# GuildOfWeavers/distaff

Hardware: AMD Instinct MI355X
Metric: trace_cells_per_sec (higher is better)
Workload: dtype u128 (prime field 2^128-45*2^40+1, 4x u32 limbs)

## Files before the change

### distaff_amd/csrc/kernels_ntt.hip

```cpp
#include "ctx.h"
#include <mutex>
#include <type_traits>
#include "ntt_lds.h"

#if defined(NTT_NO_ROTATE)
#define NTT_NO_ROTATE_DEFINED 1
#else
#define NTT_NO_ROTATE_DEFINED 0
#endif
#define NTT_TILE_ELEMS 4096

struct NttArgs {
    const fe* src; fe* dst;
    size_t src_col_stride, src_coset_stride;
    size_t dst_col_stride, dst_coset_stride;
    const fe_tw* stage_tw;
    const fe_tw* prescale;
    const fe_tw* dit_last;
    const tw4_t* tw4;
    size_t tw4_coset_stride;
    uint32_t log_n1, log_n2, tile , log_N, log_b;
    uint32_t j0;
    uint32_t has_scale;
    uint32_t tiles_per_block;
    uint32_t debug;
    size_t src_row_stride, dst_k_stride, src_batch_stride, dst_batch_stride;
    uint32_t batch_log;
    uint32_t dit;
    uint32_t groups, cosets, cols;
    uint32_t coset_fast;
    uint32_t pre;
    const fe_tw* pre_tw;
    fe_tw scale;
};

__device__ __forceinline__ fe load_fe(const fe* p) { return *p; }

__device__ __forceinline__ fe dom_pow(const fe* lo, const fe* hi, uint32_t lo_bits, uint64_t e) {
    uint32_t l = (uint32_t)e & ((1u << lo_bits) - 1u), h = (uint32_t)(e >> lo_bits);
    fe a = lo[l];
    if (h == 0) return a;
    return fe_mul(a, hi[h]);
}

__device__ __forceinline__ void ntt_block(const NttArgs& a, uint32_t& group, uint32_t& jl, uint32_t& col) {
    const uint32_t b = blockIdx.x, units = a.groups * a.cosets;
    uint32_t u;
    if (a.coset_fast) {
        const uint32_t s = b >> 3, pairs = a.cosets * a.cols, pair = s % pairs;
        group = (s / pairs) * 8u + (b & 7u);
        const uint32_t chunk = pair / (4u * a.cosets), in_chunk = pair - chunk * 4u * a.cosets;
        const uint32_t width = (chunk * 4u + 4u <= a.cols) ? 4u : a.cols - chunk * 4u;
        col = chunk * 4u + in_chunk % width; jl = in_chunk / width;
        return;
    }
    if ((units & 7u) == 0) { const uint32_t s = b >> 3; col = s % a.cols; u = (s / a.cols) * 8u + (b & 7u); }
    else { col = b % a.cols; u = b / a.cols; }
    jl = u / a.groups; group = u % a.groups;
}

struct OutB {
    static constexpr bool active = true;
    fe* __restrict__ dst ; uint32_t k_stride, log_n2; bool scale; fe_tw s;
    uint32_t pre_shift, h;
    struct Tok {};
    __device__ __forceinline__ Tok pre(uint32_t, uint32_t) const { return Tok{}; }
    __device__ __forceinline__ void put(uint32_t row, uint32_t t, const fe& v, const Tok&) const {
        const uint32_t k2 = ((log_n2 ? (__brev(row) >> (32 - log_n2)) : 0u) << pre_shift) + h;
#if NTT_STREAM_B_STORE
        fe_store_stream(dst + (k2 * k_stride + t), scale ? fe_mul_tw(v, s) : v);
#else
        dst[k2 * k_stride + t] = scale ? fe_mul_tw(v, s) : v;
#endif
    }
};

#ifndef NTT_STREAM_STORE
#define NTT_STREAM_STORE 1
#endif
#ifndef NTT_STREAM_B_STORE
#define NTT_STREAM_B_STORE 1
#endif
#ifndef NTT_STREAM_B_LOAD
#define NTT_STREAM_B_LOAD 1
#endif
#if defined(NTT_LAB_SRC_SMALL)
#define NTT_LAB_SRC(row, t, off) ((((NTT_LAB_SRC_SMALL) == 1) || hh) ? ((((row) & 1023u) << 2) + ((t) & 3u)) : (off))
#else
#define NTT_LAB_SRC(row, t, off) (off)
#endif
#if defined(NTT_LAB_TW4_SMALL)
#define NTT_LAB_TW(row, t, off) ((((row) & 1023u) << 2) + ((t) & 3u))
#else
#define NTT_LAB_TW(row, t, off) (off)
#endif
#if defined(NTT_LAB_STAMPS)
#define NTT_LAB_WG_STRIDE 61u
__device__ unsigned long long ntt_lab_buf[2 * 256 * 16 * 2 * 16];
extern "C" __attribute__((visibility("default"))) int dst_lab_stamps(unsigned long long* out, size_t count, int clear) {
    if (count > sizeof(ntt_lab_buf) / 8) return -1;
    if (hipMemcpyFromSymbol(out, HIP_SYMBOL(ntt_lab_buf), count * 8) != hipSuccess) return -2;
    if (clear) { static unsigned long long zero[2 * 256 * 16 * 2 * 16]; if (hipMemcpyToSymbol(HIP_SYMBOL(ntt_lab_buf), zero, sizeof zero) != hipSuccess) return -3; }
    return 0;
}
#define NTT_LAB_FLUSH(pass, it, st, nst) do { \
    if ((blockIdx.x % NTT_LAB_WG_STRIDE) == 0u && blockIdx.x / NTT_LAB_WG_STRIDE < 256u && (it) < 2u && (threadIdx.x & 63u) == 0u) { \
        unsigned long long* o_ = ntt_lab_buf + ((((size_t)(pass) * 256u + blockIdx.x / NTT_LAB_WG_STRIDE) * 16u + (threadIdx.x >> 6)) * 2u + (it)) * 16u; \
        for (int k_ = 0; k_ < (nst); k_++) o_[k_] = (st)[k_]; } } while (0)
#else
#define NTT_LAB_FLUSH(pass, it, st, nst) ((void)0)
#endif
extern __shared__ __attribute__((aligned(16))) unsigned char ntt_smem[];

template <int THREADS, int WPE = 4, bool PREFETCH = true, int LOG_LEN = 0, int LOG_T = 0, int PRE = 0>
__global__ void __launch_bounds__(THREADS, WPE) ntt_pass_a(NttArgs a, const fe* __restrict__ src_base, fe* __restrict__ dst_base) {
    constexpr int EPT = NTT_TILE_ELEMS / THREADS;
    fe* L = reinterpret_cast<fe*>(ntt_smem);
    const uint32_t log_n1 = LOG_LEN ? (uint32_t)LOG_LEN : a.log_n1;
    const uint32_t log_t = LOG_T ? (uint32_t)LOG_T : a.tile, T = 1u << log_t, n1 = 1u << log_n1;
    fe_tw* TW = reinterpret_cast<fe_tw*>(L + n1 * T);
    uint32_t group, jl, col;
    ntt_block(a, group, jl, col);
    uint32_t hh = 0;
    if (PRE) { const uint32_t half = a.groups >> 1; hh = group >= half ? 1u : 0u; group -= hh * half; }
    const uint32_t jg = a.j0 + jl;
    const fe* __restrict__ src0 = src_base + (size_t)col * a.src_col_stride + (size_t)jl * a.src_coset_stride;
    fe* __restrict__ dst0 = dst_base + (size_t)col * a.dst_col_stride + (size_t)jl * a.dst_coset_stride;
    const uint32_t pmask = (1u << (a.log_b + log_n1 + PRE)) - 1u;
    const uint32_t jv = jg + (hh << a.log_b);
    if (a.dit) {
        const uint32_t in_lds = a.dit_last ? n1 / 2 : n1;
        for (uint32_t i = threadIdx.x; i + 1 < in_lds; i += THREADS) {
            const uint32_t lb = 31u - (uint32_t)__clz(i + 1), k = i + 1 - (1u << lb);
            TW[i] = a.prescale[((jv + (k << (a.log_b + PRE))) << (log_n1 - lb - 1)) & pmask];
        }
    } else
    for (uint32_t i = threadIdx.x; i < n1 / 2; i += THREADS) TW[dif_tw_slot(i)] = a.stage_tw[i];
    const bool scaled = !a.dit && a.prescale != nullptr && jg != 0;
    fe pre0 = fe_zero(), pre1 = fe_zero(), pre2 = fe_zero(), pre3 = fe_zero(), pre4 = fe_zero(), pre5 = fe_zero(), pre6 = fe_zero(), pre7 = fe_zero();
    const uint32_t count = n1 * T;
#define NTT_EACH(M) { M(0, pre0) M(1, pre1) M(2, pre2) M(3, pre3) M(4, pre4) M(5, pre5) M(6, pre6) M(7, pre7) }
    const bool rot_a = a.dit && log_t == 2 && !NTT_NO_ROTATE_DEFINED;
#define NTT_COL_A(idx) (rot_a ? (((idx) + ((idx) >> log_t)) & (T - 1)) : ((idx) & (T - 1)))
    const fe_tw pre_c = (PRE && a.dit) ? a.prescale[(jg << log_n1) & pmask] : fe_tw{};
    auto pre_stage_a = [&](const fe& x0, const fe& x1, uint32_t row) -> fe {
        if (a.dit) { const fe t = fe_mul_tw(x1, pre_c); return hh ? fe_sub(x0, t) : fe_add(x0, t); }
        return hh ? fe_mul_tw(fe_sub(x0, x1), a.pre_tw[row]) : fe_add(x0, x1);
    };
#define NTT_FETCH_A1(e, var) if constexpr ((e) < EPT) { uint32_t idx = lane + (e) * THREADS; idx = idx < count ? idx : 0u; \
        if constexpr (PRE != 0) { const uint32_t row_ = idx >> log_t; const fe x0_ = src[NTT_LAB_SRC(row_, NTT_COL_A(idx), (row_ << a.log_n2) + NTT_COL_A(idx))], x1_ = src[NTT_LAB_SRC(row_ + 512u, NTT_COL_A(idx), ((row_ + n1) << a.log_n2) + NTT_COL_A(idx))]; var = pre_stage_a(x0_, x1_, row_); } \
        else var = src[NTT_LAB_SRC(idx >> log_t, NTT_COL_A(idx), ((idx >> log_t) << a.log_n2) + NTT_COL_A(idx))]; }
#define NTT_FETCH_A(tile) { const fe* __restrict__ src = src0 + (tile) * T; NTT_EACH(NTT_FETCH_A1) }
    const tw4_t* __restrict__ tw4 = a.tw4 + (size_t)jl * a.tw4_coset_stride;
    const uint32_t tile0 = group * a.tiles_per_block;
    uint32_t lane = threadIdx.x;
    if (PREFETCH) NTT_FETCH_A(tile0)
    for (uint32_t it = 0; it < a.tiles_per_block; it++) {
        const uint32_t tile = tile0 + it;
        unsigned long long st[16]; (void)st;
        NTT_STAMP_REAL(st, 14);
        NTT_STAMP(st, 8);
        lane = lds_opaque_lane();
        if (!PREFETCH) NTT_FETCH_A(tile)
        NTT_STAMP(st, 9);
        __syncthreads();
        NTT_STAMP(st, 10);
#define NTT_PUT_A(e, var) if constexpr ((e) < EPT) { const uint32_t idx = lane + (e) * THREADS; if (idx < count) { if (a.dit) L[lds_slot(__brev(idx >> log_t) >> (32 - log_n1), NTT_COL_A(idx), log_t)] = var; else L[lds_slot(idx >> log_t, idx & (T - 1), log_t)] = scaled ? fe_mul_tw(var, a.prescale[(jg * (idx >> log_t)) & pmask]) : var; } }
        NTT_EACH(NTT_PUT_A)
#undef NTT_PUT_A
        NTT_STAMP(st, 11);
        __syncthreads();
        NTT_STAMP(st, 12);
        if (PREFETCH && it + 1 < a.tiles_per_block) NTT_FETCH_A(tile + 1)
        if constexpr (LOG_LEN != 0) {
            if (a.dit) lds_ntt_dit_fixed<THREADS, LOG_LEN, LOG_T>(L, TW, a.dit_last ? a.dit_last + (size_t)((jg << PRE) + hh) * (n1 / 2) : nullptr, NttKeepInLds(), st);
            else lds_ntt_dif_fixed<THREADS, LOG_LEN, LOG_T>(L, TW, NttKeepInLds(), st);
        } else {
            if (a.dit) lds_ntt_dit<THREADS>(L, TW, log_n1, log_t, 1u, log_n1 + 1u, a.dit_last ? a.dit_last + (size_t)((jg << PRE) + hh) * (n1 / 2) : nullptr);
            else lds_ntt_dif<THREADS>(L, TW, log_n1, log_t, 1u, log_n1 + 1u);
        }
        constexpr int RB = WPE > 4 ? 1 : THREADS == 512 ? 2 : 4;
#if defined(NTT_LAB_DST_DENSE)
        fe* __restrict__ dst = dst_base + ((size_t)blockIdx.x * a.tiles_per_block + it) * count;
#else
        fe* __restrict__ dst = dst0 + tile * T;
#endif
        const tw4_t* __restrict__ tw = tw4 + tile * T;
        for (uint32_t base = 0; base < count; base += RB * THREADS) {
            fe v[RB]; tw4_t w[RB]; uint32_t off[RB]; bool ok[RB];
            static_for<0, RB>([&](auto q_) {
                constexpr int q = decltype(q_)::value;
                uint32_t idx = base + q * THREADS + lane;
                ok[q] = idx < count;
                idx = ok[q] ? idx : 0u;
                const uint32_t t = idx & (T - 1), r = idx >> log_t;
                const uint32_t k1 = ((a.dit ? r : __brev(r) >> (32 - log_n1)) << PRE) + hh;
                off[q] = (k1 << a.log_n2) + t;
                v[q] = L[idx];
                w[q] = tw[NTT_LAB_TW(r, t, off[q])];
#if defined(NTT_LAB_DST_DENSE)
                off[q] = idx;
#endif
            });
            static_for<0, RB>([&](auto q_) {
                constexpr int q = decltype(q_)::value;
#if NTT_TW4_PAIRS
                const fe out_q = fe_mul_tw(v[q], w[q]);
#else
                const fe out_q = fe_mul(v[q], w[q]);
#endif
#if NTT_STREAM_STORE
                if (ok[q]) fe_store_stream(dst + off[q], out_q);
#else
                if (ok[q]) dst[off[q]] = out_q;
#endif
            });
        }
        NTT_STAMP(st, 13);
        NTT_STAMP_REAL(st, 15);
        NTT_LAB_FLUSH(0, it, st, 16);
    }
}

template <int THREADS, int WPE = 4, bool PREFETCH = true, int LOG_LEN = 0, int LOG_T = 0, int PRE = 0>
__global__ void __launch_bounds__(THREADS, WPE) ntt_pass_b(NttArgs a, const fe* __restrict__ src_base, fe* __restrict__ dst_base) {
    constexpr int EPT = NTT_TILE_ELEMS / THREADS;
    fe* L = reinterpret_cast<fe*>(ntt_smem);
    const uint32_t log_n2 = LOG_LEN ? (uint32_t)LOG_LEN : a.log_n2;
    const uint32_t log_t = LOG_T ? (uint32_t)LOG_T : a.tile, T = 1u << log_t, n2 = 1u << log_n2;
    fe_tw* TW = reinterpret_cast<fe_tw*>(L + n2 * T);
    uint32_t g, jl, col;
    ntt_block(a, g, jl, col);
    uint32_t hh = 0;
    if (PRE) { const uint32_t half = a.groups >> 1; hh = g >= half ? 1u : 0u; g -= hh * half; }
    const uint32_t batch = g & ((1u << a.batch_log) - 1u), group = g >> a.batch_log;
    const fe* __restrict__ src = src_base + (size_t)col * a.src_col_stride + (size_t)jl * a.src_coset_stride + (size_t)batch * a.src_batch_stride;
    fe* __restrict__ dst = dst_base + (size_t)col * a.dst_col_stride + (size_t)jl * a.dst_coset_stride + (size_t)batch * a.dst_batch_stride;
    for (uint32_t i = threadIdx.x; i < n2 / 2; i += THREADS) TW[dif_tw_slot(i)] = a.stage_tw[i];
    fe pre0 = fe_zero(), pre1 = fe_zero(), pre2 = fe_zero(), pre3 = fe_zero(), pre4 = fe_zero(), pre5 = fe_zero(), pre6 = fe_zero(), pre7 = fe_zero();
    const uint32_t count = n2 * T;
    const bool colfast_b = log_t == 2 && !NTT_NO_ROTATE_DEFINED;
#define NTT_ROW_B(idx) (colfast_b ? ((idx) & (T - 1)) : ((idx) >> log_n2))
#define NTT_M2_B(idx) (colfast_b ? ((idx) >> log_t) : ((idx) & (n2 - 1)))
#if NTT_STREAM_B_LOAD
#define NTT_LOAD_B(p) fe_load_stream(p)
#else
#define NTT_LOAD_B(p) (*(p))
#endif
#define NTT_FETCH_B1(e, var) if constexpr ((e) < EPT) { uint32_t idx = lane + (e) * THREADS; idx = idx < count ? idx : 0u; \
        if constexpr (PRE != 0) { const uint32_t m_ = NTT_M2_B(idx); const fe* p_ = srct + NTT_ROW_B(idx) * row_stride + m_; const fe x0_ = p_[0], x1_ = p_[n2]; \
                                  var = hh ? fe_mul_tw(fe_sub(x0_, x1_), a.pre_tw[m_]) : fe_add(x0_, x1_); } \
        else var = NTT_LOAD_B(srct + (NTT_ROW_B(idx) * row_stride + NTT_M2_B(idx))); }
#define NTT_FETCH_B(tile) { const fe* __restrict__ srct = src + (size_t)((tile) * T) * a.src_row_stride; NTT_EACH(NTT_FETCH_B1) }
    const uint32_t row_stride = (uint32_t)a.src_row_stride;
    const uint32_t tile0 = group * a.tiles_per_block;
    uint32_t lane = threadIdx.x;
    if (PREFETCH) NTT_FETCH_B(tile0)
    for (uint32_t it = 0; it < a.tiles_per_block; it++) {
        const uint32_t k1_0 = (tile0 + it) * T;
        unsigned long long st[16]; (void)st;
        NTT_STAMP_REAL(st, 14);
        NTT_STAMP(st, 8);
        lane = lds_opaque_lane();
        if (!PREFETCH) NTT_FETCH_B(tile0 + it)
        NTT_STAMP(st, 9);
        __syncthreads();
        NTT_STAMP(st, 10);
#define NTT_PUT_B(e, var) if constexpr ((e) < EPT) { const uint32_t idx = lane + (e) * THREADS; if (idx < count) L[lds_slot(NTT_M2_B(idx), NTT_ROW_B(idx), log_t)] = var; }
        NTT_EACH(NTT_PUT_B)
#undef NTT_PUT_B
        NTT_STAMP(st, 11);
        __syncthreads();
        NTT_STAMP(st, 12);
        if (PREFETCH && it + 1 < a.tiles_per_block) NTT_FETCH_B(tile0 + it + 1)
        const OutB out{dst + k1_0, (uint32_t)a.dst_k_stride, log_n2, a.has_scale != 0, a.scale, (uint32_t)PRE, hh};
        const fe_tw* Wuse = TW;
        if constexpr (LOG_LEN != 0) lds_ntt_dif_fixed<THREADS, LOG_LEN, LOG_T, OutB>(L, Wuse, out, st);
        else lds_ntt_dif<THREADS, OutB>(L, Wuse, log_n2, log_t, 1u, log_n2 + 1u, out);
        NTT_STAMP(st, 13);
        NTT_STAMP_REAL(st, 15);
        NTT_LAB_FLUSH(1, it, st, 16);
    }
}

template <int LOGL> struct NttDigits;
template <> struct NttDigits<6>  { static constexpr int r1 = 3, r2 = 3, r3 = 0, log_t = 2; };
template <> struct NttDigits<7>  { static constexpr int r1 = 4, r2 = 3, r3 = 0, log_t = 2; };
template <> struct NttDigits<8>  { static constexpr int r1 = 4, r2 = 4, r3 = 0, log_t = 2; };
template <> struct NttDigits<9>  { static constexpr int r1 = 3, r2 = 3, r3 = 3, log_t = 2; };
template <> struct NttDigits<10> { static constexpr int r1 = 4, r2 = 3, r3 = 3, log_t = 2; };
template <> struct NttDigits<11> { static constexpr int r1 = 4, r2 = 4, r3 = 3, log_t = 2; };
template <> struct NttDigits<12> { static constexpr int r1 = 4, r2 = 4, r3 = 4, log_t = 1; };

struct NttRegArgs {
    const fe* src; fe* dst;
    size_t src_col_stride, src_coset_stride, dst_col_stride, dst_coset_stride;
    size_t in_stride_m, in_stride_t;
    size_t out_stride_k;
    const fe_tw* stage_tw;
    const fe* tw_lo; const fe* tw_hi;
    const fe_tw* prescale;
    uint32_t lo_bits, log_N, log_b, j0, coset_twiddle, has_scale;
    fe scale;
    fe c16[8];
};

constexpr __host__ __device__ int ntt_brev(int v, int bits) { int r = 0; for (int i = 0; i < bits; i++) r |= ((v >> i) & 1) << (bits - 1 - i); return r; }

__device__ __attribute__((noinline)) fe fe_mul_call(fe a, fe b) { return fe_mul(a, b); }
__device__ __attribute__((noinline)) fe fe_mul_tw_call(fe a, fe p, fe q) { return fe_mul_tw(a, p, q); }

template <int r>
__device__ __forceinline__ void dft_regs(fe* x, const fe* c16) {
    constexpr int R = 1 << r;
    static_for<0, r>([&](auto s_) {
        constexpr int s = decltype(s_)::value, half = R >> (s + 1);
        static_for<0, R / 2>([&](auto i_) {
            constexpr int i = decltype(i_)::value, b = (i / half) * 2 * half, j = i % half;
            fe u = x[b + j], v = x[b + j + half];
            x[b + j] = fe_add(u, v);
            fe d = fe_sub(u, v);
            if constexpr (j == 0) x[b + j + half] = d;
            else x[b + j + half] = fe_mul_call(d, c16[(j << s) << (4 - r)]);
        });
    });
}

template <int LOGL>
__device__ __forceinline__ fe mul_stage_twiddle(const fe& v, const fe_tw* __restrict__ tw, uint32_t e) {
    constexpr uint32_t H = 1u << (LOGL - 1);
    const fe_tw w = tw[e & (H - 1)];
    const fe r = fe_mul_tw_call(v, w.p, w.q);
    return (e & H) ? fe_neg(r) : r;
}

template <int LOGL>
__global__ void __launch_bounds__((1 << (LOGL + NttDigits<LOGL>::log_t)) / 16, (LOGL + NttDigits<LOGL>::log_t >= 13) ? 1 : 2) ntt_reg_kernel(NttRegArgs a) {
    using D = NttDigits<LOGL>;
    constexpr int r1 = D::r1, r2 = D::r2, r3 = D::r3, LT = D::log_t, T = 1 << LT;
    constexpr int rq = r3 ? r3 : r2;
// ... 154 lines not shown
    (void)hipFuncSetAttribute((const void*)ntt_pass_b<1024>, hipFuncAttributeMaxDynamicSharedMemorySize, 160 * 1024);
    (void)hipFuncSetAttribute((const void*)ntt_pass_a<1024, 8, false>, hipFuncAttributeMaxDynamicSharedMemorySize, 160 * 1024);
    (void)hipFuncSetAttribute((const void*)ntt_pass_a<1024, 8, false, 10, 2>, hipFuncAttributeMaxDynamicSharedMemorySize, 160 * 1024);
    (void)hipFuncSetAttribute((const void*)ntt_pass_a<1024, 8, false, 8, 4>, hipFuncAttributeMaxDynamicSharedMemorySize, 160 * 1024);
    (void)hipFuncSetAttribute((const void*)ntt_pass_b<1024, 8, false, 8, 4>, hipFuncAttributeMaxDynamicSharedMemorySize, 160 * 1024);
    (void)hipFuncSetAttribute((const void*)ntt_pass_a<512, 4, true, 8, 4>, hipFuncAttributeMaxDynamicSharedMemorySize, 160 * 1024);
    (void)hipFuncSetAttribute((const void*)ntt_pass_b<512, 4, true, 8, 4>, hipFuncAttributeMaxDynamicSharedMemorySize, 160 * 1024);
    (void)hipFuncSetAttribute((const void*)ntt_pass_b<1024, 8, true, 10, 2>, hipFuncAttributeMaxDynamicSharedMemorySize, 160 * 1024);
    (void)hipFuncSetAttribute((const void*)ntt_pass_b<1024, 8, false>, hipFuncAttributeMaxDynamicSharedMemorySize, 160 * 1024);
    (void)hipFuncSetAttribute((const void*)ntt_pass_a<1024, 8, false, 10, 2, 1>, hipFuncAttributeMaxDynamicSharedMemorySize, 160 * 1024);
    (void)hipFuncSetAttribute((const void*)ntt_pass_b<1024, 8, false, 10, 2, 1>, hipFuncAttributeMaxDynamicSharedMemorySize, 160 * 1024);
    (void)hipFuncSetAttribute((const void*)ntt_pass_a<512, 4, true, 0, 0, 1>, hipFuncAttributeMaxDynamicSharedMemorySize, 160 * 1024);
    (void)hipFuncSetAttribute((const void*)ntt_pass_b<512, 4, true, 0, 0, 1>, hipFuncAttributeMaxDynamicSharedMemorySize, 160 * 1024);

    raised[c->device] = true;
}
static void ntt_report_occupancy(const char* name, bool pass_b, int threads, bool eight, size_t lds) {
    static std::mutex mu;
    static std::map<std::string, bool> seen;
    char key[128]; snprintf(key, sizeof key, "%s/%d/%d/%zu", name, threads, (int)eight, lds);
    std::lock_guard<std::mutex> lock(mu);
    if (seen[key]) return; seen[key] = true;
    int nb = -1;
    hipError_t e;
    if (eight) e = pass_b ? hipOccupancyMaxActiveBlocksPerMultiprocessor(&nb, ntt_pass_b<1024, 8, false>, 1024, lds) : hipOccupancyMaxActiveBlocksPerMultiprocessor(&nb, ntt_pass_a<1024, 8, false>, 1024, lds);
    else if (threads == 512) e = pass_b ? hipOccupancyMaxActiveBlocksPerMultiprocessor(&nb, ntt_pass_b<512>, 512, lds) : hipOccupancyMaxActiveBlocksPerMultiprocessor(&nb, ntt_pass_a<512>, 512, lds);
    else e = pass_b ? hipOccupancyMaxActiveBlocksPerMultiprocessor(&nb, ntt_pass_b<1024>, 1024, lds) : hipOccupancyMaxActiveBlocksPerMultiprocessor(&nb, ntt_pass_a<1024>, 1024, lds);
    fprintf(stderr, "[distaff] %s: %d lanes, %zu B LDS -> %d workgroups per CU (%s)\n", name, threads, lds, nb, hipGetErrorString(e));
}
#define NTT_LDS_TWO_PER_CU (80 * 1024)
static void ntt_launch(dst_ctx* c, bool pass_b, NttArgs& a, size_t groups, size_t cosets, size_t cols, size_t lds, const char* name, double bytes) {
    ntt_raise_lds_limit(c);
    a.groups = (uint32_t)groups; a.cosets = (uint32_t)cosets; a.cols = (uint32_t)cols;
    const dim3 grid((unsigned)(groups * cosets * cols));
    const uint32_t stages = pass_b ? a.log_n2 : a.log_n1;
    double mults = (!pass_b && a.dit) ? 0.5 * stages : ((stages & 1u) ? 0.5 * (stages - 1) : (stages >= 2 ? 0.5 * stages - 0.75 : 0.0));
    if (!pass_b) mults += ((!a.dit && a.prescale != nullptr) ? 1.0 : 0.0) + (NTT_TW4_PAIRS ? 1.0 : 21.0 / 18.0); else if (a.has_scale) mults += 1.0;
    if (a.pre) mults += (!pass_b && a.dit) ? 1.0 : 0.5;
    const double elements = (double)groups * a.tiles_per_block * ((size_t)1 << a.tile) * ((size_t)1 << stages) * cosets * cols;
    KScope ks_(c, name, bytes, true, 18.0 * mults * elements);
    const char* wv = c->sw("DISTAFF_NTT_WAVES");
    const bool two = lds <= NTT_LDS_TWO_PER_CU, eight = two && (wv ? wv[0] == '8' : stages >= 10);
    const bool any_shape = c->sw_is("DISTAFF_NTT_FIXED", "0");
    const bool fixed = stages == 10 && a.tile == 2 && !any_shape;
    const bool fixed84 = stages == 8 && a.tile == 4 && !any_shape;
    if (a.debug & 1u) ntt_report_occupancy(name, pass_b, eight || !two ? 1024 : 512, eight, lds);
    if (a.pre) {
        if (pass_b && fixed) hipLaunchKernelGGL((ntt_pass_b<1024, 8, false, 10, 2, 1>), grid, dim3(1024), lds, c->stream, a, a.src, a.dst);
        else if (!pass_b && fixed) hipLaunchKernelGGL((ntt_pass_a<1024, 8, false, 10, 2, 1>), grid, dim3(1024), lds, c->stream, a, a.src, a.dst);
        else if (pass_b) hipLaunchKernelGGL((ntt_pass_b<512, 4, true, 0, 0, 1>), grid, dim3(512), lds, c->stream, a, a.src, a.dst);
        else hipLaunchKernelGGL((ntt_pass_a<512, 4, true, 0, 0, 1>), grid, dim3(512), lds, c->stream, a, a.src, a.dst);
        return;
    }
    if (two) {
        if (pass_b && eight && fixed) hipLaunchKernelGGL((ntt_pass_b<1024, 8, true, 10, 2>), grid, dim3(1024), lds, c->stream, a, a.src, a.dst);
        else if (!pass_b && eight && fixed) hipLaunchKernelGGL((ntt_pass_a<1024, 8, false, 10, 2>), grid, dim3(1024), lds, c->stream, a, a.src, a.dst);
        else if (pass_b && eight && fixed84) hipLaunchKernelGGL((ntt_pass_b<1024, 8, false, 8, 4>), grid, dim3(1024), lds, c->stream, a, a.src, a.dst);
        else if (!pass_b && eight && fixed84) hipLaunchKernelGGL((ntt_pass_a<1024, 8, false, 8, 4>), grid, dim3(1024), lds, c->stream, a, a.src, a.dst);
        else if (pass_b && fixed84) hipLaunchKernelGGL((ntt_pass_b<512, 4, true, 8, 4>), grid, dim3(512), lds, c->stream, a, a.src, a.dst);
        else if (!pass_b && fixed84) hipLaunchKernelGGL((ntt_pass_a<512, 4, true, 8, 4>), grid, dim3(512), lds, c->stream, a, a.src, a.dst);
        else if (pass_b && eight) hipLaunchKernelGGL((ntt_pass_b<1024, 8, false>), grid, dim3(1024), lds, c->stream, a, a.src, a.dst);
        else if (pass_b) hipLaunchKernelGGL(ntt_pass_b<512>, grid, dim3(512), lds, c->stream, a, a.src, a.dst);
        else if (eight) hipLaunchKernelGGL((ntt_pass_a<1024, 8, false>), grid, dim3(1024), lds, c->stream, a, a.src, a.dst);
        else hipLaunchKernelGGL(ntt_pass_a<512>, grid, dim3(512), lds, c->stream, a, a.src, a.dst);
    } else {
        if (pass_b) hipLaunchKernelGGL(ntt_pass_b<1024>, grid, dim3(1024), lds, c->stream, a, a.src, a.dst);
// ... 371 lines not shown
```

### distaff_amd/csrc/ntt_lds.h

```cpp
#pragma once
#include <type_traits>
#include "fe.h"

template <int I, int N, class F>
__device__ __forceinline__ void static_for(F&& f) {
    if constexpr (I < N) { f(std::integral_constant<int, I>{}); static_for<I + 1, N>(f); }
}

__device__ __forceinline__ uint32_t lds_slot(uint32_t i, uint32_t t, uint32_t log_t) {
#if defined(NTT_SWIZZLE)
    if (log_t == 2) return ((i ^ ((i >> 2) & 3u)) << 2) + (t ^ ((i >> 1) & 3u));
#endif
    return (i << log_t) + t;
}

__device__ __forceinline__ uint32_t lds_column(uint32_t w, uint32_t q, uint32_t log_t, bool adjacent_rows) {
    const uint32_t T = 1u << log_t;
#if !defined(NTT_NO_ROTATE)
    if (adjacent_rows && log_t == 2) return (w + q) & (T - 1);
#endif
    return w & (T - 1);
}

__device__ __forceinline__ constexpr bool lds_wave_local() {
#if defined(NTT_NO_WAVE_LOCAL)
    return false;
#else
    return true;
#endif
}

__device__ __forceinline__ void lds_wave_sync() {
#if defined(__HIP_DEVICE_COMPILE__)
#if !defined(__gfx950__)
#error "the rows a wavefront owns (own_rows in the rounds below) are counted for the 64-lane wavefronts of gfx950"
#endif
    asm volatile("" ::: "memory");
    __builtin_amdgcn_wave_barrier();
    asm volatile("" ::: "memory");
#else
    __syncthreads();
#endif
}

__device__ __forceinline__ uint32_t dif_tw_slot(uint32_t e) {
    return e ^ ((e >> 3) & 7u) ^ ((e >> 6) & 7u);
}

__device__ __forceinline__ uint32_t lds_opaque_lane() {
    uint32_t lane = threadIdx.x;
#if defined(__HIP_DEVICE_COMPILE__)
    asm volatile("" : "+v"(lane));
#endif
    return lane;
}
#if defined(NTT_LAB_STAMPS) && defined(__HIP_DEVICE_COMPILE__)
#define NTT_STAMP(arr, k) ((arr)[k] = __builtin_readcyclecounter())
#define NTT_STAMP_REAL(arr, k) ((arr)[k] = wall_clock64())
#else
#define NTT_STAMP(arr, k) ((void)0)
#define NTT_STAMP_REAL(arr, k) ((void)0)
#endif

struct NttKeepInLds {
    static constexpr bool active = false;
    struct Tok {};
    __device__ __forceinline__ Tok pre(uint32_t, uint32_t) const { return Tok{}; }
    __device__ __forceinline__ void put(uint32_t, uint32_t, const fe&, const Tok&) const {}
};

template <int THREADS, class Out>
__device__ __forceinline__ void lds_dif_round(fe* L, const fe_tw* W, uint32_t log_len, uint32_t log_t, uint32_t s, const Out& out, uint32_t lane) {
    const uint32_t T = 1u << log_t;
    const uint32_t ld = log_len - s;
    const uint32_t d = 1u << ld, hd = d >> 1;
    const bool last = (s + 1 == log_len);
    const bool fin = Out::active && last;
    for (uint32_t w = lane; w < ((1u << log_len) >> 2) * T; w += THREADS) {
        const uint32_t q = w >> log_t;
        const uint32_t t = lds_column(w, q, log_t, hd == 1);
        const uint32_t pos = q & (hd - 1), blk = q >> (ld - 1);
        const uint32_t i0 = (blk << (ld + 1)) + pos;
        typename Out::Tok k0, k1, k2, k3;
        if (fin) { k0 = out.pre(i0, t); k1 = out.pre(i0 + hd, t); k2 = out.pre(i0 + d, t); k3 = out.pre(i0 + d + hd, t); }
        fe* p0 = L + lds_slot(i0, t, log_t); fe* p1 = L + lds_slot(i0 + hd, t, log_t); fe* p2 = L + lds_slot(i0 + d, t, log_t); fe* p3 = L + lds_slot(i0 + d + hd, t, log_t);
        const fe x0 = *p0, x1 = *p1, x2 = *p2, x3 = *p3;
        fe a0, a1, a2, a3;
        fe_addsub(x0, x2, a0, a2);
        fe_addsub(x1, x3, a1, a3);
#define NTT_TW_AT(idx) W[dif_tw_slot(idx)]
        if (hd != 1) a2 = fe_mul_tw(a2, NTT_TW_AT(pos << (s - 1)));
        a3 = fe_mul_tw(a3, NTT_TW_AT((pos + hd) << (s - 1)));
        fe y0, y1, y2, y3;
        fe_addsub(a0, a1, y0, y1);
        fe_addsub(a2, a3, y2, y3);
        if (!last && hd != 1) { const fe_tw tw = NTT_TW_AT(pos << s); y1 = fe_mul_tw(y1, tw); y3 = fe_mul_tw(y3, tw); }
#undef NTT_TW_AT
        if (fin) { out.put(i0, t, y0, k0); out.put(i0 + hd, t, y1, k1); out.put(i0 + d, t, y2, k2); out.put(i0 + d + hd, t, y3, k3); }
        else { *p0 = y0; *p1 = y1; *p2 = y2; *p3 = y3; }
    }
    const bool own_rows = lds_wave_local() && (2u << ld) <= ((64u >> log_t) << 2) && s + 3 <= log_len;
    if (!fin) { if (own_rows) lds_wave_sync(); else __syncthreads(); }
}
template <int THREADS, class Out>
__device__ __forceinline__ void lds_dif_tail(fe* L, uint32_t log_len, uint32_t log_t, const Out& out, uint32_t lane) {
    const uint32_t T = 1u << log_t;
    for (uint32_t w = lane; w < ((1u << log_len) >> 1) * T; w += THREADS) {
        const uint32_t t = w & (T - 1), q = w >> log_t;
        typename Out::Tok k0, k1;
        if (Out::active) { k0 = out.pre(q << 1, t); k1 = out.pre((q << 1) + 1, t); }
        fe* p0 = L + lds_slot(q << 1, t, log_t); fe* p1 = L + lds_slot((q << 1) + 1, t, log_t);
        const fe a = *p0, b = *p1;
        fe sum, dif;
        fe_addsub(a, b, sum, dif);
        if (Out::active) { out.put(q << 1, t, sum, k0); out.put((q << 1) + 1, t, dif, k1); }
        else { *p0 = sum; *p1 = dif; }
    }
    if (!Out::active) __syncthreads();
}
template <int THREADS, class Out = NttKeepInLds>
__device__ __forceinline__ void lds_ntt_dif(fe* L, const fe_tw* W, uint32_t log_len, uint32_t log_t, uint32_t s_from, uint32_t s_to, const Out& out = Out()) {
    uint32_t s = s_from;
    const uint32_t lane = lds_opaque_lane();
    for (; s + 1 <= log_len && s < s_to; s += 2) lds_dif_round<THREADS, Out>(L, W, log_len, log_t, s, out, lane);
    if (s == log_len && s < s_to) lds_dif_tail<THREADS, Out>(L, log_len, log_t, out, lane);
}
template <int THREADS, int LOG_LEN, int LOG_T, class Out = NttKeepInLds>
__device__ __forceinline__ void lds_ntt_dif_fixed(fe* L, const fe_tw* W, const Out& out = Out(), unsigned long long* stamps = nullptr) {
    const uint32_t lane = lds_opaque_lane();
    static_for<0, LOG_LEN / 2>([&](auto r_) { constexpr uint32_t s = 1u + 2u * decltype(r_)::value; lds_dif_round<THREADS, Out>(L, W, (uint32_t)LOG_LEN, (uint32_t)LOG_T, s, out, lane); (void)stamps; NTT_STAMP(stamps, decltype(r_)::value); });
    if constexpr (LOG_LEN & 1) lds_dif_tail<THREADS, Out>(L, (uint32_t)LOG_LEN, (uint32_t)LOG_T, out, lane);
}

template <int THREADS, class Out>
__device__ __forceinline__ void lds_dit_round(fe* L, const fe_tw* W, uint32_t log_len, uint32_t log_t, uint32_t s, const fe_tw* __restrict__ Wlast, const Out& out, uint32_t lane) {
    const uint32_t T = 1u << log_t;
    const uint32_t B = 1u << s, half = B >> 1;
    const bool fin = Out::active && s + 1 == log_len;
    for (uint32_t w = lane; w < ((1u << log_len) >> 2) * T; w += THREADS) {
        const uint32_t q = w >> log_t;
        const uint32_t t = lds_column(w, q, log_t, half == 1);
        const uint32_t k = q & (half - 1), base = (q >> (s - 1)) << (s + 1);
        typename Out::Tok k0, k1, k2, k3;
        if (fin) { k0 = out.pre(base + k, t); k1 = out.pre(base + k + half, t); k2 = out.pre(base + k + B, t); k3 = out.pre(base + k + B + half, t); }
        fe* p0 = L + lds_slot(base + k, t, log_t); fe* p1 = L + lds_slot(base + k + half, t, log_t); fe* p2 = L + lds_slot(base + k + B, t, log_t); fe* p3 = L + lds_slot(base + k + B + half, t, log_t);
        const fe_tw tb = W[half - 1 + k];
        const fe x0 = *p0, x1 = fe_mul_tw(*p1, tb), x2 = *p2, x3 = fe_mul_tw(*p3, tb);
        fe a0, a1, b2, b3;
        fe_addsub(x0, x1, a0, a1);
        fe_addsub(x2, x3, b2, b3);
        const bool from_global = Wlast != nullptr && s + 1 == log_len;
        const fe_tw t2 = from_global ? Wlast[k] : W[B - 1 + k], t3 = from_global ? Wlast[k + half] : W[B - 1 + k + half];
        const fe a2 = fe_mul_tw(b2, t2), a3 = fe_mul_tw(b3, t3);
        fe y0, y1, y2, y3;
        fe_addsub(a0, a2, y0, y2);
        fe_addsub(a1, a3, y1, y3);
        if (fin) { out.put(base + k, t, y0, k0); out.put(base + k + B, t, y2, k2); out.put(base + k + half, t, y1, k1); out.put(base + k + B + half, t, y3, k3); }
        else { *p0 = y0; *p2 = y2; *p1 = y1; *p3 = y3; }
    }
    const bool own_rows = lds_wave_local() && (8u << s) <= ((64u >> log_t) << 2) && s + 3 <= log_len;
    if (!fin) { if (own_rows) lds_wave_sync(); else __syncthreads(); }
}
template <int THREADS, class Out>
__device__ __forceinline__ void lds_dit_tail(fe* L, const fe_tw* W, uint32_t log_len, uint32_t log_t, const fe_tw* __restrict__ Wlast, const Out& out, uint32_t lane) {
    const uint32_t T = 1u << log_t;
    const uint32_t half = 1u << (log_len - 1);
    for (uint32_t w = lane; w < half * T; w += THREADS) {
        const uint32_t t = w & (T - 1), k = w >> log_t;
        typename Out::Tok k0, k1;
        if (Out::active) { k0 = out.pre(k, t); k1 = out.pre(k + half, t); }
        fe* p0 = L + lds_slot(k, t, log_t); fe* p1 = L + lds_slot(k + half, t, log_t);
        const fe u = *p0, v = fe_mul_tw(*p1, Wlast != nullptr ? Wlast[k] : W[half - 1 + k]);
        fe sum, dif;
        fe_addsub(u, v, sum, dif);
        if (Out::active) { out.put(k, t, sum, k0); out.put(k + half, t, dif, k1); }
        else { *p0 = sum; *p1 = dif; }
    }
    if (!Out::active) __syncthreads();
}
template <int THREADS, class Out = NttKeepInLds>
__device__ __forceinline__ void lds_ntt_dit(fe* L, const fe_tw* W, uint32_t log_len, uint32_t log_t, uint32_t s_from, uint32_t s_to, const fe_tw* __restrict__ Wlast = nullptr, const Out& out = Out()) {
    uint32_t s = s_from;
    const uint32_t lane = lds_opaque_lane();
    for (; s + 1 <= log_len && s < s_to; s += 2) lds_dit_round<THREADS, Out>(L, W, log_len, log_t, s, Wlast, out, lane);
    if (s == log_len && s < s_to) lds_dit_tail<THREADS, Out>(L, W, log_len, log_t, Wlast, out, lane);
}
template <int THREADS, int LOG_LEN, int LOG_T, class Out = NttKeepInLds>
__device__ __forceinline__ void lds_ntt_dit_fixed(fe* L, const fe_tw* W, const fe_tw* __restrict__ Wlast = nullptr, const Out& out = Out(), unsigned long long* stamps = nullptr) {
    const uint32_t lane = lds_opaque_lane();
    static_for<0, LOG_LEN / 2>([&](auto r_) { constexpr uint32_t s = 1u + 2u * decltype(r_)::value; lds_dit_round<THREADS, Out>(L, W, (uint32_t)LOG_LEN, (uint32_t)LOG_T, s, Wlast, out, lane); (void)stamps; NTT_STAMP(stamps, decltype(r_)::value); });
    if constexpr (LOG_LEN & 1) lds_dit_tail<THREADS, Out>(L, W, (uint32_t)LOG_LEN, (uint32_t)LOG_T, Wlast, out, lane);
}
```

Before: 603.1 million.

## Cut NTT integer address arithmetic with magic division and 32-bit byte offsets

Replaces runtime integer divisions and modulos in block-index decoding with precomputed multiply-shift reciprocals computed on the host. Global addressing in both NTT passes switches to 32-bit byte offsets built from log2 strides. Fixed-shape kernels get specialised fetch, LDS-put and twiddle-store paths that hoist per-lane offsets and drop bounds checks. The output token now carries a base offset, so each butterfly computes only a bit-reversed delta, and lane bounds are asserted to the compiler. This trims scalar and vector ALU work around memory-bound passes, at the risk of 32-bit offset overflow on very large strides.

New measurement: 605.8 million, median of 3. About the same (+0.5%).

```diff
diff --git a/distaff_amd/csrc/kernels_ntt.hip b/distaff_amd/csrc/kernels_ntt.hip
--- a/distaff_amd/csrc/kernels_ntt.hip
+++ b/distaff_amd/csrc/kernels_ntt.hip
@@ -9,6 +9,17 @@
 #define NTT_NO_ROTATE_DEFINED 0
 #endif
 #define NTT_TILE_ELEMS 4096
+
+struct NttDiv { uint32_t mul, shift , d; };
+static NttDiv ntt_div_make(uint32_t d) {
+    NttDiv r{0u, 0u, d ? d : 1u};
+    if (r.d < 2) return r;
+    uint32_t l = 0; while (((uint64_t)1 << l) < r.d) l++;
+    r.mul = (uint32_t)((((uint64_t)1 << (31 + l)) + r.d - 1) / r.d); r.shift = l - 1;
+    return r;
+}
+__host__ __device__ __forceinline__ uint32_t ntt_div(uint32_t x, const NttDiv& v) { return v.mul ? (uint32_t)(((uint64_t)x * v.mul) >> 32) >> v.shift : x; }
+__host__ __device__ __forceinline__ uint32_t ntt_mod(uint32_t x, const NttDiv& v) { return x - ntt_div(x, v) * v.d; }
 
 struct NttArgs {
     const fe* src; fe* dst;
@@ -29,6 +40,8 @@
     uint32_t dit;
     uint32_t groups, cosets, cols;
     uint32_t coset_fast;
+    NttDiv div_groups, div_cols, div_pairs , div_chunk , div_tail ;
+    uint32_t dst_k_log, src_row_log;
     uint32_t pre;
     const fe_tw* pre_tw;
     fe_tw scale;
@@ -47,30 +60,45 @@
     const uint32_t b = blockIdx.x, units = a.groups * a.cosets;
     uint32_t u;
     if (a.coset_fast) {
-        const uint32_t s = b >> 3, pairs = a.cosets * a.cols, pair = s % pairs;
-        group = (s / pairs) * 8u + (b & 7u);
-        const uint32_t chunk = pair / (4u * a.cosets), in_chunk = pair - chunk * 4u * a.cosets;
-        const uint32_t width = (chunk * 4u + 4u <= a.cols) ? 4u : a.cols - chunk * 4u;
-        col = chunk * 4u + in_chunk % width; jl = in_chunk / width;
+        const uint32_t s = b >> 3, sp = ntt_div(s, a.div_pairs), pair = s - sp * a.div_pairs.d;
+        group = sp * 8u + (b & 7u);
+        const uint32_t chunk = ntt_div(pair, a.div_chunk), in_chunk = pair - chunk * a.div_chunk.d;
+        if (chunk * 4u + 4u <= a.cols) { col = chunk * 4u + (in_chunk & 3u); jl = in_chunk >> 2; }
+        else { jl = ntt_div(in_chunk, a.div_tail); col = chunk * 4u + (in_chunk - jl * a.div_tail.d); }
         return;
     }
-    if ((units & 7u) == 0) { const uint32_t s = b >> 3; col = s % a.cols; u = (s / a.cols) * 8u + (b & 7u); }
-    else { col = b % a.cols; u = b / a.cols; }
-    jl = u / a.groups; group = u % a.groups;
-}
+    if ((units & 7u) == 0) { const uint32_t s = b >> 3, sc = ntt_div(s, a.div_cols); col = s - sc * a.div_cols.d; u = sc * 8u + (b & 7u); }
+    else { u = ntt_div(b, a.div_cols); col = b - u * a.div_cols.d; }
+    jl = ntt_div(u, a.div_groups); group = u - jl * a.div_groups.d;
+}
+template <class X>
+__device__ __forceinline__ X* ntt_at(X* base, uint32_t byte_off) {
+    typedef typename std::conditional<std::is_const<X>::value, const char, char>::type byte_t;
+    return reinterpret_cast<X*>(reinterpret_cast<byte_t*>(base) + byte_off);
+}
+#if defined(NTT_LAB_SRC_SMALL) || defined(NTT_LAB_TW4_SMALL) || defined(NTT_LAB_DST_DENSE)
+#define NTT_LAB_ADDR 1
+#else
+#define NTT_LAB_ADDR 0
+#endif
+constexpr __host__ __device__ int ntt_brev(int v, int bits) { int r = 0; for (int i = 0; i < bits; i++) r |= ((v >> i) & 1) << (bits - 1 - i); return r; }
+
 
 struct OutB {
     static constexpr bool active = true;
-    fe* __restrict__ dst ; uint32_t k_stride, log_n2; bool scale; fe_tw s;
+    fe* __restrict__ dst ; uint32_t k_log , log_n2; bool scale; fe_tw s;
     uint32_t pre_shift, h;
-    struct Tok {};
-    __device__ __forceinline__ Tok pre(uint32_t, uint32_t) const { return Tok{}; }
-    __device__ __forceinline__ void put(uint32_t row, uint32_t t, const fe& v, const Tok&) const {
-        const uint32_t k2 = ((log_n2 ? (__brev(row) >> (32 - log_n2)) : 0u) << pre_shift) + h;
+    struct Tok { uint32_t off; };
+    __device__ __forceinline__ Tok at(uint32_t row0, uint32_t t) const {
+        return Tok{(log_n2 ? (__brev(row0) >> (28u - log_n2 - pre_shift - k_log)) : 0u) + (t << 4)};
+    }
+    __device__ __forceinline__ void put(const Tok& k, uint32_t j, const fe& v) const {
+        const uint32_t kj = ((log_n2 ? (__brev(j) >> (32u - log_n2)) : 0u) << pre_shift) + h;
+        fe* p = ntt_at(dst, k.off + ((kj << k_log) << 4));
 #if NTT_STREAM_B_STORE
-        fe_store_stream(dst + (k2 * k_stride + t), scale ? fe_mul_tw(v, s) : v);
-#else
-        dst[k2 * k_stride + t] = scale ? fe_mul_tw(v, s) : v;
+        fe_store_stream(p, scale ? fe_mul_tw(v, s) : v);
+#else
+        *p = scale ? fe_mul_tw(v, s) : v;
 #endif
     }
 };
@@ -118,6 +146,9 @@
     fe* L = reinterpret_cast<fe*>(ntt_smem);
     const uint32_t log_n1 = LOG_LEN ? (uint32_t)LOG_LEN : a.log_n1;
     const uint32_t log_t = LOG_T ? (uint32_t)LOG_T : a.tile, T = 1u << log_t, n1 = 1u << log_n1;
+    constexpr bool FIXA = LOG_LEN != 0 && !NTT_LAB_ADDR;
+    constexpr uint32_t RS = (uint32_t)THREADS >> LOG_T;
+    static_assert(LOG_LEN == 0 || ((1 << (LOG_LEN + LOG_T)) == NTT_TILE_ELEMS && THREADS % (16 << LOG_T) == 0), "fixed shapes fill the tile; the column rotation needs whole groups of four rows per step");
     fe_tw* TW = reinterpret_cast<fe_tw*>(L + n1 * T);
     uint32_t group, jl, col;
     ntt_block(a, group, jl, col);
@@ -147,10 +178,13 @@
         if (a.dit) { const fe t = fe_mul_tw(x1, pre_c); return hh ? fe_sub(x0, t) : fe_add(x0, t); }
         return hh ? fe_mul_tw(fe_sub(x0, x1), a.pre_tw[row]) : fe_add(x0, x1);
     };
-#define NTT_FETCH_A1(e, var) if constexpr ((e) < EPT) { uint32_t idx = lane + (e) * THREADS; idx = idx < count ? idx : 0u; \
+#define NTT_FETCH_A1(e, var) if constexpr ((e) < EPT && FIXA) { const uint32_t oe_ = voff_ + ((((e) * RS) << a.log_n2) << 4); \
+        if constexpr (PRE != 0) { const fe x0_ = *ntt_at(src, oe_), x1_ = *ntt_at(src, oe_ + ((n1 << a.log_n2) << 4)); var = pre_stage_a(x0_, x1_, (lane >> log_t) + (e) * RS); } \
+        else var = *ntt_at(src, oe_); } \
+    else if constexpr ((e) < EPT) { uint32_t idx = lane + (e) * THREADS; idx = idx < count ? idx : 0u; \
         if constexpr (PRE != 0) { const uint32_t row_ = idx >> log_t; const fe x0_ = src[NTT_LAB_SRC(row_, NTT_COL_A(idx), (row_ << a.log_n2) + NTT_COL_A(idx))], x1_ = src[NTT_LAB_SRC(row_ + 512u, NTT_COL_A(idx), ((row_ + n1) << a.log_n2) + NTT_COL_A(idx))]; var = pre_stage_a(x0_, x1_, row_); } \
         else var = src[NTT_LAB_SRC(idx >> log_t, NTT_COL_A(idx), ((idx >> log_t) << a.log_n2) + NTT_COL_A(idx))]; }
-#define NTT_FETCH_A(tile) { const fe* __restrict__ src = src0 + (tile) * T; NTT_EACH(NTT_FETCH_A1) }
+#define NTT_FETCH_A(tile) { const fe* __restrict__ src = src0 + (tile) * T; const uint32_t voff_ = (((lane >> log_t) << a.log_n2) + NTT_COL_A(lane)) << 4; (void)voff_; NTT_EACH(NTT_FETCH_A1) }
     const tw4_t* __restrict__ tw4 = a.tw4 + (size_t)jl * a.tw4_coset_stride;
     const uint32_t tile0 = group * a.tiles_per_block;
     uint32_t lane = threadIdx.x;
@@ -160,12 +194,12 @@
         unsigned long long st[16]; (void)st;
         NTT_STAMP_REAL(st, 14);
         NTT_STAMP(st, 8);
-        lane = lds_opaque_lane();
+        lane = lds_opaque_lane<THREADS>();
         if (!PREFETCH) NTT_FETCH_A(tile)
         NTT_STAMP(st, 9);
         __syncthreads();
         NTT_STAMP(st, 10);
-#define NTT_PUT_A(e, var) if constexpr ((e) < EPT) { const uint32_t idx = lane + (e) * THREADS; if (idx < count) { if (a.dit) L[lds_slot(__brev(idx >> log_t) >> (32 - log_n1), NTT_COL_A(idx), log_t)] = var; else L[lds_slot(idx >> log_t, idx & (T - 1), log_t)] = scaled ? fe_mul_tw(var, a.prescale[(jg * (idx >> log_t)) & pmask]) : var; } }
+#define NTT_PUT_A(e, var) if constexpr ((e) < EPT) { const uint32_t idx = lane + (e) * THREADS; if (FIXA || idx < count) { if (a.dit) L[lds_slot(FIXA ? (__brev(lane >> log_t) >> (32 - log_n1)) + (uint32_t)ntt_brev((int)((e) * RS), LOG_LEN) : __brev(idx >> log_t) >> (32 - log_n1), NTT_COL_A(FIXA ? lane : idx), log_t)] = var; else L[lds_slot(idx >> log_t, idx & (T - 1), log_t)] = scaled ? fe_mul_tw(var, a.prescale[(jg * (idx >> log_t)) & pmask]) : var; } }
         NTT_EACH(NTT_PUT_A)
 #undef NTT_PUT_A
         NTT_STAMP(st, 11);
@@ -186,6 +220,35 @@
         fe* __restrict__ dst = dst0 + tile * T;
 #endif
         const tw4_t* __restrict__ tw = tw4 + tile * T;
+        if constexpr (FIXA) {
+            const uint32_t t = lane & (T - 1), r0 = lane >> log_t;
+            const uint32_t voff = ((((a.dit ? r0 : __brev(r0) >> (32 - log_n1)) << PRE) << a.log_n2) + t) << 4;
+#pragma unroll 1
+            for (uint32_t e0 = 0; e0 < (uint32_t)EPT; e0 += RB) {
+                fe v[RB]; tw4_t w[RB]; uint32_t off[RB];
+                static_for<0, RB>([&](auto q_) {
+                    constexpr int q = decltype(q_)::value;
+                    const uint32_t e = e0 + q;
+                    const uint32_t ke = ((a.dit ? e * RS : __brev(e * RS) >> (32 - LOG_LEN)) << PRE) + hh;
+                    off[q] = voff + ((ke << a.log_n2) << 4);
+                    v[q] = L[lane + e * THREADS];
+                    w[q] = *ntt_at(tw, off[q] * (uint32_t)(sizeof(tw4_t) / 16));
+                });
+                static_for<0, RB>([&](auto q_) {
+                    constexpr int q = decltype(q_)::value;
+#if NTT_TW4_PAIRS
+                    const fe out_q = fe_mul_tw(v[q], w[q]);
+#else
+                    const fe out_q = fe_mul(v[q], w[q]);
+#endif
+#if NTT_STREAM_STORE
+                    fe_store_stream(ntt_at(dst, off[q]), out_q);
+#else
+                    *ntt_at(dst, off[q]) = out_q;
+#endif
+                });
+            }
+        } else
         for (uint32_t base = 0; base < count; base += RB * THREADS) {
             fe v[RB]; tw4_t w[RB]; uint32_t off[RB]; bool ok[RB];
             static_for<0, RB>([&](auto q_) {
@@ -228,6 +291,8 @@
     fe* L = reinterpret_cast<fe*>(ntt_smem);
     const uint32_t log_n2 = LOG_LEN ? (uint32_t)LOG_LEN : a.log_n2;
     const uint32_t log_t = LOG_T ? (uint32_t)LOG_T : a.tile, T = 1u << log_t, n2 = 1u << log_n2;
+    constexpr bool FIXB = LOG_LEN != 0 && !NTT_LAB_ADDR;
+    static_assert(LOG_LEN == 0 || ((1 << (LOG_LEN + LOG_T)) == NTT_TILE_ELEMS && THREADS % (1 << LOG_T) == 0 && THREADS % (1 << LOG_LEN) == 0), "fixed shapes fill the tile");
     fe_tw* TW = reinterpret_cast<fe_tw*>(L + n2 * T);
     uint32_t g, jl, col;
     ntt_block(a, g, jl, col);
@@ -247,11 +312,15 @@
 #else
 #define NTT_LOAD_B(p) (*(p))
 #endif
-#define NTT_FETCH_B1(e, var) if constexpr ((e) < EPT) { uint32_t idx = lane + (e) * THREADS; idx = idx < count ? idx : 0u; \
+#define NTT_FETCH_B1(e, var) if constexpr ((e) < EPT && FIXB) { const uint32_t oe_ = voff_ + (((NTT_ROW_B((e) * THREADS) << a.src_row_log) + NTT_M2_B((e) * THREADS)) << 4); \
+        if constexpr (PRE != 0) { const fe x0_ = *ntt_at(srct, oe_), x1_ = *ntt_at(srct, oe_ + (n2 << 4)); \
+                                  var = hh ? fe_mul_tw(fe_sub(x0_, x1_), a.pre_tw[NTT_M2_B(lane) + NTT_M2_B((e) * THREADS)]) : fe_add(x0_, x1_); } \
+        else var = NTT_LOAD_B(ntt_at(srct, oe_)); } \
+    else if constexpr ((e) < EPT) { uint32_t idx = lane + (e) * THREADS; idx = idx < count ? idx : 0u; \
         if constexpr (PRE != 0) { const uint32_t m_ = NTT_M2_B(idx); const fe* p_ = srct + NTT_ROW_B(idx) * row_stride + m_; const fe x0_ = p_[0], x1_ = p_[n2]; \
                                   var = hh ? fe_mul_tw(fe_sub(x0_, x1_), a.pre_tw[m_]) : fe_add(x0_, x1_); } \
         else var = NTT_LOAD_B(srct + (NTT_ROW_B(idx) * row_stride + NTT_M2_B(idx))); }
-#define NTT_FETCH_B(tile) { const fe* __restrict__ srct = src + (size_t)((tile) * T) * a.src_row_stride; NTT_EACH(NTT_FETCH_B1) }
+#define NTT_FETCH_B(tile) { const fe* __restrict__ srct = src + (size_t)((tile) * T) * a.src_row_stride; const uint32_t voff_ = ((NTT_ROW_B(lane) << a.src_row_log) + NTT_M2_B(lane)) << 4; (void)voff_; NTT_EACH(NTT_FETCH_B1) }
     const uint32_t row_stride = (uint32_t)a.src_row_stride;
     const uint32_t tile0 = group * a.tiles_per_block;
     uint32_t lane = threadIdx.x;
@@ -261,19 +330,20 @@
         unsigned long long st[16]; (void)st;
         NTT_STAMP_REAL(st, 14);
         NTT_STAMP(st, 8);
-        lane = lds_opaque_lane();
+        lane = lds_opaque_lane<THREADS>();
         if (!PREFETCH) NTT_FETCH_B(tile0 + it)
         NTT_STAMP(st, 9);
         __syncthreads();
         NTT_STAMP(st, 10);
-#define NTT_PUT_B(e, var) if constexpr ((e) < EPT) { const uint32_t idx = lane + (e) * THREADS; if (idx < count) L[lds_slot(NTT_M2_B(idx), NTT_ROW_B(idx), log_t)] = var; }
+#define NTT_PUT_B(e, var) if constexpr ((e) < EPT && FIXB) L[lds_slot(NTT_M2_B(lane) + NTT_M2_B((e) * THREADS), NTT_ROW_B(lane) + NTT_ROW_B((e) * THREADS), log_t)] = var; \
+    else if constexpr ((e) < EPT) { const uint32_t idx = lane + (e) * THREADS; if (idx < count) L[lds_slot(NTT_M2_B(idx), NTT_ROW_B(idx), log_t)] = var; }
         NTT_EACH(NTT_PUT_B)
 #undef NTT_PUT_B
         NTT_STAMP(st, 11);
         __syncthreads();
         NTT_STAMP(st, 12);
         if (PREFETCH && it + 1 < a.tiles_per_block) NTT_FETCH_B(tile0 + it + 1)
-        const OutB out{dst + k1_0, (uint32_t)a.dst_k_stride, log_n2, a.has_scale != 0, a.scale, (uint32_t)PRE, hh};
+        const OutB out{dst + k1_0, a.dst_k_log, log_n2, a.has_scale != 0, a.scale, (uint32_t)PRE, hh};
         const fe_tw* Wuse = TW;
         if constexpr (LOG_LEN != 0) lds_ntt_dif_fixed<THREADS, LOG_LEN, LOG_T, OutB>(L, Wuse, out, st);
         else lds_ntt_dif<THREADS, OutB>(L, Wuse, log_n2, log_t, 1u, log_n2 + 1u, out);
@@ -304,8 +374,6 @@
     fe scale;
     fe c16[8];
 };
-
-constexpr __host__ __device__ int ntt_brev(int v, int bits) { int r = 0; for (int i = 0; i < bits; i++) r |= ((v >> i) & 1) << (bits - 1 - i); return r; }
 
 __device__ __attribute__((noinline)) fe fe_mul_call(fe a, fe b) { return fe_mul(a, b); }
 __device__ __attribute__((noinline)) fe fe_mul_tw_call(fe a, fe p, fe q) { return fe_mul_tw(a, p, q); }
@@ -526,6 +594,10 @@
 static void ntt_launch(dst_ctx* c, bool pass_b, NttArgs& a, size_t groups, size_t cosets, size_t cols, size_t lds, const char* name, double bytes) {
     ntt_raise_lds_limit(c);
     a.groups = (uint32_t)groups; a.cosets = (uint32_t)cosets; a.cols = (uint32_t)cols;
+    a.div_groups = ntt_div_make(a.groups); a.div_cols = ntt_div_make(a.cols); a.div_pairs = ntt_div_make(a.cosets * a.cols);
+    a.div_chunk = ntt_div_make(4u * a.cosets); a.div_tail = ntt_div_make(a.cols & 3u);
+    a.src_row_log = pass_b ? (uint32_t)__builtin_ctzll((unsigned long long)a.src_row_stride) : 0u;
+    a.dst_k_log = pass_b ? (uint32_t)__builtin_ctzll((unsigned long long)a.dst_k_stride) : 0u;
     const dim3 grid((unsigned)(groups * cosets * cols));
     const uint32_t stages = pass_b ? a.log_n2 : a.log_n1;
     double mults = (!pass_b && a.dit) ? 0.5 * stages : ((stages & 1u) ? 0.5 * (stages - 1) : (stages >= 2 ? 0.5 * stages - 0.75 : 0.0));
diff --git a/distaff_amd/csrc/ntt_lds.h b/distaff_amd/csrc/ntt_lds.h
--- a/distaff_amd/csrc/ntt_lds.h
+++ b/distaff_amd/csrc/ntt_lds.h
@@ -47,10 +47,12 @@
     return e ^ ((e >> 3) & 7u) ^ ((e >> 6) & 7u);
 }
 
+template <int THREADS = 0>
 __device__ __forceinline__ uint32_t lds_opaque_lane() {
     uint32_t lane = threadIdx.x;
 #if defined(__HIP_DEVICE_COMPILE__)
     asm volatile("" : "+v"(lane));
+    if constexpr (THREADS != 0) __builtin_assume(lane < (uint32_t)THREADS);
 #endif
     return lane;
 }
@@ -65,8 +67,8 @@
 struct NttKeepInLds {
     static constexpr bool active = false;
     struct Tok {};
-    __device__ __forceinline__ Tok pre(uint32_t, uint32_t) const { return Tok{}; }
-    __device__ __forceinline__ void put(uint32_t, uint32_t, const fe&, const Tok&) const {}
+    __device__ __forceinline__ Tok at(uint32_t, uint32_t) const { return Tok{}; }
+    __device__ __forceinline__ void put(const Tok&, uint32_t, const fe&) const {}
 };
 
 template <int THREADS, class Out>
@@ -81,8 +83,6 @@
         const uint32_t t = lds_column(w, q, log_t, hd == 1);
         const uint32_t pos = q & (hd - 1), blk = q >> (ld - 1);
         const uint32_t i0 = (blk << (ld + 1)) + pos;
-        typename Out::Tok k0, k1, k2, k3;
-        if (fin) { k0 = out.pre(i0, t); k1 = out.pre(i0 + hd, t); k2 = out.pre(i0 + d, t); k3 = out.pre(i0 + d + hd, t); }
         fe* p0 = L + lds_slot(i0, t, log_t); fe* p1 = L + lds_slot(i0 + hd, t, log_t); fe* p2 = L + lds_slot(i0 + d, t, log_t); fe* p3 = L + lds_slot(i0 + d + hd, t, log_t);
         const fe x0 = *p0, x1 = *p1, x2 = *p2, x3 = *p3;
         fe a0, a1, a2, a3;
@@ -96,7 +96,7 @@
         fe_addsub(a2, a3, y2, y3);
         if (!last && hd != 1) { const fe_tw tw = NTT_TW_AT(pos << s); y1 = fe_mul_tw(y1, tw); y3 = fe_mul_tw(y3, tw); }
 #undef NTT_TW_AT
-        if (fin) { out.put(i0, t, y0, k0); out.put(i0 + hd, t, y1, k1); out.put(i0 + d, t, y2, k2); out.put(i0 + d + hd, t, y3, k3); }
+        if (fin) { const typename Out::Tok k = out.at(i0, t); out.put(k, 0u, y0); out.put(k, hd, y1); out.put(k, d, y2); out.put(k, d + hd, y3); }
         else { *p0 = y0; *p1 = y1; *p2 = y2; *p3 = y3; }
     }
     const bool own_rows = lds_wave_local() && (2u << ld) <= ((64u >> log_t) << 2) && s + 3 <= log_len;
@@ -107,13 +107,11 @@
     const uint32_t T = 1u << log_t;
     for (uint32_t w = lane; w < ((1u << log_len) >> 1) * T; w += THREADS) {
         const uint32_t t = w & (T - 1), q = w >> log_t;
-        typename Out::Tok k0, k1;
-        if (Out::active) { k0 = out.pre(q << 1, t); k1 = out.pre((q << 1) + 1, t); }
         fe* p0 = L + lds_slot(q << 1, t, log_t); fe* p1 = L + lds_slot((q << 1) + 1, t, log_t);
         const fe a = *p0, b = *p1;
         fe sum, dif;
         fe_addsub(a, b, sum, dif);
-        if (Out::active) { out.put(q << 1, t, sum, k0); out.put((q << 1) + 1, t, dif, k1); }
+        if (Out::active) { const typename Out::Tok k = out.at(q << 1, t); out.put(k, 0u, sum); out.put(k, 1u, dif); }
         else { *p0 = sum; *p1 = dif; }
     }
     if (!Out::active) __syncthreads();
@@ -121,13 +119,13 @@
 template <int THREADS, class Out = NttKeepInLds>
 __device__ __forceinline__ void lds_ntt_dif(fe* L, const fe_tw* W, uint32_t log_len, uint32_t log_t, uint32_t s_from, uint32_t s_to, const Out& out = Out()) {
     uint32_t s = s_from;
-    const uint32_t lane = lds_opaque_lane();
+    const uint32_t lane = lds_opaque_lane<THREADS>();
     for (; s + 1 <= log_len && s < s_to; s += 2) lds_dif_round<THREADS, Out>(L, W, log_len, log_t, s, out, lane);
     if (s == log_len && s < s_to) lds_dif_tail<THREADS, Out>(L, log_len, log_t, out, lane);
 }
 template <int THREADS, int LOG_LEN, int LOG_T, class Out = NttKeepInLds>
 __device__ __forceinline__ void lds_ntt_dif_fixed(fe* L, const fe_tw* W, const Out& out = Out(), unsigned long long* stamps = nullptr) {
-    const uint32_t lane = lds_opaque_lane();
+    const uint32_t lane = lds_opaque_lane<THREADS>();
     static_for<0, LOG_LEN / 2>([&](auto r_) { constexpr uint32_t s = 1u + 2u * decltype(r_)::value; lds_dif_round<THREADS, Out>(L, W, (uint32_t)LOG_LEN, (uint32_t)LOG_T, s, out, lane); (void)stamps; NTT_STAMP(stamps, decltype(r_)::value); });
     if constexpr (LOG_LEN & 1) lds_dif_tail<THREADS, Out>(L, (uint32_t)LOG_LEN, (uint32_t)LOG_T, out, lane);
 }
@@ -141,8 +139,6 @@
         const uint32_t q = w >> log_t;
         const uint32_t t = lds_column(w, q, log_t, half == 1);
         const uint32_t k = q & (half - 1), base = (q >> (s - 1)) << (s + 1);
-        typename Out::Tok k0, k1, k2, k3;
-        if (fin) { k0 = out.pre(base + k, t); k1 = out.pre(base + k + half, t); k2 = out.pre(base + k + B, t); k3 = out.pre(base + k + B + half, t); }
         fe* p0 = L + lds_slot(base + k, t, log_t); fe* p1 = L + lds_slot(base + k + half, t, log_t); fe* p2 = L + lds_slot(base + k + B, t, log_t); fe* p3 = L + lds_slot(base + k + B + half, t, log_t);
         const fe_tw tb = W[half - 1 + k];
         const fe x0 = *p0, x1 = fe_mul_tw(*p1, tb), x2 = *p2, x3 = fe_mul_tw(*p3, tb);
@@ -155,7 +151,7 @@
         fe y0, y1, y2, y3;
         fe_addsub(a0, a2, y0, y2);
         fe_addsub(a1, a3, y1, y3);
-        if (fin) { out.put(base + k, t, y0, k0); out.put(base + k + B, t, y2, k2); out.put(base + k + half, t, y1, k1); out.put(base + k + B + half, t, y3, k3); }
+        if (fin) { const typename Out::Tok kk = out.at(base + k, t); out.put(kk, 0u, y0); out.put(kk, B, y2); out.put(kk, half, y1); out.put(kk, B + half, y3); }
         else { *p0 = y0; *p2 = y2; *p1 = y1; *p3 = y3; }
     }
     const bool own_rows = lds_wave_local() && (8u << s) <= ((64u >> log_t) << 2) && s + 3 <= log_len;
@@ -167,13 +163,11 @@
     const uint32_t half = 1u << (log_len - 1);
     for (uint32_t w = lane; w < half * T; w += THREADS) {
         const uint32_t t = w & (T - 1), k = w >> log_t;
-        typename Out::Tok k0, k1;
-        if (Out::active) { k0 = out.pre(k, t); k1 = out.pre(k + half, t); }
         fe* p0 = L + lds_slot(k, t, log_t); fe* p1 = L + lds_slot(k + half, t, log_t);
         const fe u = *p0, v = fe_mul_tw(*p1, Wlast != nullptr ? Wlast[k] : W[half - 1 + k]);
         fe sum, dif;
         fe_addsub(u, v, sum, dif);
-        if (Out::active) { out.put(k, t, sum, k0); out.put(k + half, t, dif, k1); }
+        if (Out::active) { const typename Out::Tok kk = out.at(k, t); out.put(kk, 0u, sum); out.put(kk, half, dif); }
         else { *p0 = sum; *p1 = dif; }
     }
     if (!Out::active) __syncthreads();
@@ -181,13 +175,13 @@
 template <int THREADS, class Out = NttKeepInLds>
 __device__ __forceinline__ void lds_ntt_dit(fe* L, const fe_tw* W, uint32_t log_len, uint32_t log_t, uint32_t s_from, uint32_t s_to, const fe_tw* __restrict__ Wlast = nullptr, const Out& out = Out()) {
     uint32_t s = s_from;
-    const uint32_t lane = lds_opaque_lane();
+    const uint32_t lane = lds_opaque_lane<THREADS>();
     for (; s + 1 <= log_len && s < s_to; s += 2) lds_dit_round<THREADS, Out>(L, W, log_len, log_t, s, Wlast, out, lane);
     if (s == log_len && s < s_to) lds_dit_tail<THREADS, Out>(L, W, log_len, log_t, Wlast, out, lane);
 }
 template <int THREADS, int LOG_LEN, int LOG_T, class Out = NttKeepInLds>
 __device__ __forceinline__ void lds_ntt_dit_fixed(fe* L, const fe_tw* W, const fe_tw* __restrict__ Wlast = nullptr, const Out& out = Out(), unsigned long long* stamps = nullptr) {
-    const uint32_t lane = lds_opaque_lane();
+    const uint32_t lane = lds_opaque_lane<THREADS>();
     static_for<0, LOG_LEN / 2>([&](auto r_) { constexpr uint32_t s = 1u + 2u * decltype(r_)::value; lds_dit_round<THREADS, Out>(L, W, (uint32_t)LOG_LEN, (uint32_t)LOG_T, s, Wlast, out, lane); (void)stamps; NTT_STAMP(stamps, decltype(r_)::value); });
     if constexpr (LOG_LEN & 1) lds_dit_tail<THREADS, Out>(L, W, (uint32_t)LOG_LEN, (uint32_t)LOG_T, Wlast, out, lane);
 }
```
